# DAGroup-PKU/MHLA

Measured on AMD Instinct MI355X. Metric: MHLA fwd+bwd tokens/sec at (B,N,H,D), higher is better.
Workload: dtype bf16; 1 GPU; block-mix MHLA op fwd+bwd, per GPU B=8 N=4096 H=16 D=64 M=64 S=64 bf16 (BASELINE.json configs[1]); global_batch=8, parallelism=dp1 (batch shards, dW all-reduce only)

## Files before the change

### mhla_amd/csrc/capi_bm_typed.hpp

```cpp
#pragma once
#include "capi_common.hpp"
#include "blockmix.hpp"
#include "split.hpp"
#include "split16.hpp"
#include "mixh2.hpp"

namespace mhla {
namespace capi {

static_assert(sp::mixr_te<4, true>() == mixr_slice(true) && sp::mixr_te<4, false>() == mixr_slice(false), "bm_plan's resident-mixing rule");
template <int DT> constexpr int sp_state_threads() {
#ifdef MHLA_SP_STATE_4WAVES
    return NTHREADS;
#else
    return DT == 8 ? 512 : NTHREADS;
#endif
}
#ifndef SP_MIXH2_IH
#define SP_MIXH2_IH 2
#endif
#ifndef SP_MIXH2_RT
#define SP_MIXH2_RT 1
#endif

// ... 112 lines not shown
            break;
        case K_SP_MIXH: case K_SP_MIXH2:
            if constexpr (P24OK) return sp_mixh<TRANS>(o, p.mix[TRANS], p.nw, TRANS && p.dw_fused, wz, name, parts);
            break;
        default: break;
    }
    return fail(MHLA_EINVAL, "%s is not built for this type / head dim", name);
}
template <int TRANS>
int launch_wz(const float* W, int ldw, const float* x, float* out, int BH, int M, int S, float eps, hipStream_t st) {
    return launch(k_wz<TRANS>, dim3((S + 63) / 64, (M + 63) / 64, BH), dim3(NTHREADS), 0, st, N_WZ[TRANS], W, ldw, x, out, M, S, eps);
}

template <typename ET, int DT, int TRANS, bool S16>
int bm_state(const BmPlan& p, const BmCall& c, const StateArgs& a) {
    constexpr bool F32 = std::is_same<ET, float>::value;
    constexpr int SNT = sp_state_threads<DT>();
    const dim3 g(c.M, c.B * c.H);
    const char* name = p.n_state[TRANS];
    if (p.state == K_BM_STATE) return launch(k_bm_state<ET, DT, TRANS>, g, dim3(NTHREADS), state_smem_floats<DT>() * 4, c.st, name, a);
    if (p.state == K_S16_STATE) return launch(s16::k_s16_state<TRANS>, dim3((c.M + s16::WPB - 1) / s16::WPB, c.B * c.H), dim3(64 * s16::WPB), s16::state_smem(), c.st, name, a);
    if (p.rope) {
        if (p.fmt == SF_P24 || p.fmt == SF_H16) {
            if constexpr (F32 && bm_p24_built<ET, DT, S16>()) return launch(sp::k_sp_state<ET, DT, TRANS, true, SNT, false, 1>, g, dim3(SNT), sp::sp_state_smem<DT>(), c.st, name, a);
        } else if constexpr (F32 || TRANS == 0)
            return launch(sp::k_sp_state<ET, DT, TRANS, true, SNT, S16>, g, dim3(SNT), sp::sp_state_smem<DT>(), c.st, name, a);
        return MHLA_OK;
    }
    if constexpr (TRANS == 0 && bm_h16_built<ET, DT, S16>()) {
        if (p.fmt == SF_H16 && !(c.normalize && c.split) && g_recut.load())
            return launch(sp::k_sp_state<ET, DT, 0, false, SNT, S16, 2, false, false>, g, dim3(SNT), sp::sp_state_smem<DT>(), c.st, name, a);
    }
    WITH_PF(p.fmt, return launch(sp::k_sp_state<ET, DT, TRANS, false, SNT, S16, PF>, g, dim3(SNT),
                                 (PF && TRANS && sizeof(ET) == 2 && DT <= 4) ? sp::sp_state_rd_smem<DT>() : sp::sp_state_smem<DT>(), c.st, name, a));
    return MHLA_OK;
}
template <typename ET, int DT, bool S16>
int bm_state_and_mix(const BmPlan& p, const BmCall& c) {
    const BmWs& w = c.w;
    StateArgs a{};
    a.rcos = c.rcos; a.rsin = c.rsin; a.ldr = c.ldr;
    a.x = cv(c.k_num); a.y = cv(c.v); a.kd = cv(c.k_den); a.qd = cv(c.q_den); a.idx = c.block_index;
    a.out = w.kv; a.ksum = w.ksum; a.zo = w.z; a.es = w.es;
    a.H = c.H; a.M = c.M; a.S = c.S; a.D = c.D; a.eps = c.eps; a.relu = c.relu(); a.normalize = c.normalize; a.split = c.split;
    RC((bm_state<ET, DT, 0, S16>(p, c, a)));
    RC((bm_mix<0, S16, bm_p24_built<ET, DT, S16>()>(p, c)));
    if (p.wz_kernel) RC(launch_wz<0>(c.W, c.ldw, w.z, w.ninv, c.B * c.H, c.M, c.S, c.eps, c.st));
    return MHLA_OK;
}

template <typename ET, int DT, bool S16, typename TO = ET, bool EPI = false>
int sp_out(const BmPlan& p, const BmCall& c, const OutArgs& o, const char* name) {
    if constexpr (!EPI && bm_h16_built<ET, DT, S16>() && DT <= 4) {
        if (p.fmt == SF_H16 && bm_one_tile(c.S))
            return launch(sp::k_sp_out<ET, DT, TO, false, S16, 2, false, false, true>, dim3(c.M, c.B * c.H), dim3(sp::SP_OUT_T), sp::sp_out_smem<DT, S16>(), c.st, name, o);
    }
    WITH_PF(p.fmt, return launch(sp::k_sp_out<ET, DT, TO, EPI, S16, PF>, dim3(c.M, c.B * c.H), dim3(sp::SP_OUT_T), sp::sp_out_smem<DT, S16>(), c.st, name, o));
    return MHLA_OK;
}
inline OutArgs out_args(const BmCall& c) {
    OutArgs o{};
    o.rcos = c.rcos; o.rsin = c.rsin; o.ldr = c.ldr;
    o.q = cv(c.q_num); o.idx = c.block_index; o.W = c.W; o.ldw = c.ldw; o.g = c.w.g; o.ninv = c.w.ninv;
    o.H = c.H; o.M = c.M; o.S = c.S; o.D = c.D; o.eps = c.eps; o.es = c.w.es; o.relu = c.relu(); o.normalize = c.normalize;
    return o;
}
template <typename ET, int DT, bool S16>
// ... 48 lines not shown
    *parts = BH * nsplit;
    const DwArgs d{w.dg, w.kv, E, nullptr, nullptr, 0, w.dwp, M, tiles, nsplit, w.es};
    const dim3 g(p.dw_v ? 1 : tiles * tiles, BH, nsplit);
    if (p.dw == K_SP_DWT) {
        if constexpr (P24OK) return launch(sp::k_sp_dwt<true>, g, dim3(NTHREADS), sp::SP_DWT_SMEM, c.st, p.n_dw, d);
        return fail(MHLA_EINVAL, "%s is not built for this type / head dim", p.n_dw);
    }
    if (p.dw_v == 16) return launch(sp::k_sp_dw<S16, 1>, g, dim3(NTHREADS), sp::SP_DW_SMEM, c.st, p.n_dw, d);
    if (p.dw_v == 32) return launch(sp::k_sp_dw<S16, 2>, g, dim3(NTHREADS), sp::SP_DW_SMEM, c.st, p.n_dw, d);
    return launch(sp::k_sp_dw<S16>, g, dim3(NTHREADS), sp::SP_DW_SMEM, c.st, p.n_dw, d);
}
template <int MASK = 0>
int launch_dnz(const BmCall& c, int tiles, int parts) {
    const DwArgs dzz{c.w.dn, c.w.z, (long)c.S, nullptr, nullptr, 0, c.w.dwp + (size_t)parts * c.M * c.M, c.M, tiles, 1};
    return launch(k_dw<MASK>, dim3(tiles * tiles, c.B * c.H, 1), dim3(NTHREADS), DW_SMEM_FLOATS * 4, c.st, N_DNZ, dzz);
}
template <int MASK = 0>
int launch_dw_reduce(const float* dwp, float* dW, int M, int parts, int BH, bool el16, hipStream_t st) {
    if (el16 || M * M <= 1024 || parts >= 128) return launch(k_dw_reduce<MASK, 16>, dim3((M * M + 15) / 16), dim3(256), 0, st, N_DW_REDUCE, dwp, (const float*)nullptr, dW, M, M, parts, BH);
    return launch(k_dw_reduce<MASK>, dim3((M * M + 63) / 64), dim3(256), 0, st, N_DW_REDUCE, dwp, (const float*)nullptr, dW, M, M, parts, BH);
}

template <typename ET, int DT, bool S16>
int bm_tok(const BmPlan& p, const BmCall& c, const TokArgs& t) {
    const dim3 g(c.M, c.B * c.H), blk(NTHREADS);
    if (p.tok == K_BM_TOK) return launch(k_bm_bwd_tok<ET, DT>, g, blk, tok_smem_floats<DT>() * 4, c.st, p.n_tok[0], t);
    if (p.tok == K_S16_TOK) {
        const dim3 g16((c.M + s16::WPB - 1) / s16::WPB, c.B * c.H), b16(64 * s16::WPB);
        RC(launch(s16::k_s16_bwd_dq<0>, g16, b16, 0, c.st, p.n_tok[0], t));
        return launch(s16::k_s16_bwd_dkv<0>, g16, b16, s16::dkv_smem(), c.st, p.n_tok[1], t);
    }
    if (p.rope) {
        if constexpr (std::is_same<ET, float>::value) {
            WITH_PF(p.fmt, RC(launch(sp::k_sp_bwd_dq<ET, DT, true, false, false, PF>, g, blk, sp::sp_tok_smem<DT, false>(), c.st, p.n_tok[0], t));
                           return launch(sp::k_sp_bwd_dkv<ET, DT, true, false, PF>, g, blk, sp::sp_tok_smem<DT, false>(), c.st, p.n_tok[1], t));
        }
        return MHLA_OK;
    }
    const bool wq = c.normalize && !c.relu() && sizeof(ET) == 2 && DT != 5;
    constexpr bool ONE_BUILT = bm_h16_built<ET, DT, S16>() && DT <= 4;
    if (wq && ONE_BUILT && p.fmt == SF_H16 && bm_one_tile(c.S)) {
        if constexpr (ONE_BUILT) RC(launch(sp::k_sp_bwd_dq<ET, DT, false, S16, true, 2, true>, g, blk, sp::sp_tok_smem<DT, S16>(), c.st, p.n_tok[0], t));
    } else if (wq) WITH_PF(p.fmt, RC(launch(sp::k_sp_bwd_dq<ET, DT, false, S16, true, PF>, g, blk, sp::sp_tok_smem<DT, S16>(), c.st, p.n_tok[0], t)));
    else WITH_PF(p.fmt, RC(launch(sp::k_sp_bwd_dq<ET, DT, false, S16, false, PF>, g, blk, sp::sp_tok_smem<DT, S16>(), c.st, p.n_tok[0], t)));
    WITH_PF(p.fmt, return launch(sp::k_sp_bwd_dkv<ET, DT, false, S16, PF>, g, blk, sp::sp_tok_smem<DT, S16>(), c.st, p.n_tok[1], t));
    return MHLA_OK;
}

template <typename ET, bool S16>
int bm_fwd_typed(const BmCall& c) {
    const BmPlan p = bm_plan(c, false);
    DISPATCH_DT(dt_for(c.D), {
        RC((bm_state_and_mix<ET, DT, S16>(p, c)));
        OutArgs o = out_args(c);
        o.o = cmv(c.out);
        o.olo = (c.normalize && !c.epi && !(c.flags & MHLA_FLAG_NO_BWD_STATE)) ? c.w.olo : nullptr;
        RC((bm_out<ET, DT, S16>(p, c, o, p.n_out)));
    });
    return MHLA_OK;
}

template <typename ET, bool S16>
int bm_bwd_typed(const BmCall& c) {
    const BmPlan p = bm_plan(c, true);
    const BmWs& w = c.w;
    const int BH = c.B * c.H, M = c.M, S = c.S, tiles = (M + 63) / 64;
    DISPATCH_DT(dt_for(c.D), {
        if (!c.reuse) RC((bm_state_and_mix<ET, DT, S16>(p, c)));
        const bool want_olo = c.normalize && w.olo != nullptr, own_olo = !c.reuse || (c.flags & MHLA_FLAG_NO_BWD_STATE);
        if (want_olo && own_olo) {
            OutArgs o = out_args(c);
            o.o = MView{nullptr, 0, 0, 0}; o.olo = c.olo_own; o.skip_out = 1;
            RC((bm_out<ET, DT, S16>(p, c, o, p.n_olo)));
        }
        StateArgs a{};
        a.x = cv(c.q_num); a.y = cv(c.dout); a.o = cv(c.outv); a.idx = c.block_index; a.W = c.W; a.ldw = c.ldw; a.ninv = w.ninv;
        a.out = w.dg; a.dn = w.dn; a.es = w.es; a.H = c.H; a.M = M; a.S = S; a.D = c.D; a.eps = c.eps;
// ... 30 lines not shown
```

### mhla_amd/csrc/common.hpp

```cpp
#pragma once
#include <hip/hip_runtime.h>
#include <stdint.h>

namespace mhla {

typedef float f32x4 __attribute__((ext_vector_type(4)));
typedef float f32x2 __attribute__((ext_vector_type(2)));

struct bf16_t { unsigned short v; };
struct f16_t { _Float16 v; };

__device__ __forceinline__ float bf16_to_f32(unsigned short h) { return __uint_as_float(((unsigned)h) << 16); }
__device__ __forceinline__ unsigned short f32_to_bf16(float f) {
    unsigned u = __float_as_uint(f);
    if ((u & 0x7fffffffu) > 0x7f800000u) return (unsigned short)((u >> 16) | 0x40);
    u += 0x7fffu + ((u >> 16) & 1u);
    return (unsigned short)(u >> 16);
}

typedef __bf16 bf16x2_t __attribute__((ext_vector_type(2)));
__device__ __forceinline__ unsigned pack_bf16x2(float lo, float hi) {
    f32x2 v = {lo, hi};
    return __builtin_bit_cast(unsigned, __builtin_convertvector(v, bf16x2_t));
}
// ... 105 lines not shown

__device__ __forceinline__ float h16_mult_from_max(float mx) {
    const unsigned e = (__float_as_uint(mx) >> 23) & 0xffu;
    return __uint_as_float((e < 15u ? 1u : (e > 254u ? 240u : e - 14u)) << 23);
}
__device__ __forceinline__ float h16_mult_from_bound(float beta) {
    unsigned f = (__float_as_uint(beta) + 0x7fffffu) >> 23;
    f = f < 1u ? 1u : (f > 253u ? 253u : f);
    return __uint_as_float(f << 23);
}
__device__ __forceinline__ float h16_inv(float m) { return __uint_as_float(0x7f000000u - __float_as_uint(m)); }
typedef _Float16 h16x2_t __attribute__((ext_vector_type(2)));
__device__ __forceinline__ unsigned h16_pack2(float a, float b) {
    const h16x2_t h = {(_Float16)a, (_Float16)b};
    return __builtin_bit_cast(unsigned, h);
}
__device__ __forceinline__ uint4 h16_pack8(const f32x4& a, const f32x4& b, float inv) {
    return make_uint4(h16_pack2(a[0] * inv, a[1] * inv), h16_pack2(a[2] * inv, a[3] * inv), h16_pack2(b[0] * inv, b[1] * inv), h16_pack2(b[2] * inv, b[3] * inv));
}
__device__ __forceinline__ void h16_split8(const uint4& pay, float m, uint4& hi, uint4& lo) {
    const unsigned w[4] = {pay.x, pay.y, pay.z, pay.w};
    unsigned h[4], l[4];
#pragma unroll
    for (int j = 0; j < 4; ++j) {
        const h16x2_t p = __builtin_bit_cast(h16x2_t, w[j]);
        const float x0 = (float)p[0] * m, x1 = (float)p[1] * m;
        const unsigned u0 = __float_as_uint(x0), u1 = __float_as_uint(x1);
        h[j] = __builtin_amdgcn_perm(u1, u0, 0x07060302u);
        const float d0 = x0 - __uint_as_float(u0 & 0xffff0000u), d1 = x1 - __uint_as_float(u1 & 0xffff0000u);
        l[j] = __builtin_amdgcn_perm(__float_as_uint(d1), __float_as_uint(d0), 0x07060302u);
    }
    hi = make_uint4(h[0], h[1], h[2], h[3]);
    lo = make_uint4(l[0], l[1], l[2], l[3]);
}

struct View {
    const void* ptr;
    long sb, sn, sh;
};
struct MView {
    void* ptr;
    long sb, sn, sh;
};

__host__ __device__ constexpr int ld_kmajor(int dp) { return ((dp + 15) / 32) * 32 + 16; }
__host__ __device__ constexpr int ld_xmajor(int dp) { return dp + 2; }

__device__ __forceinline__ f32x4 mfma4(float a, float b, f32x4 c) {
    return __builtin_amdgcn_mfma_f32_16x16x4f32(a, b, c, 0, 0, 0);
}

__device__ __forceinline__ float wave_sum(float v) {
#pragma unroll
    for (int o = 32; o > 0; o >>= 1) v += __shfl_xor(v, o, 64);
    return v;
}

__device__ __forceinline__ float row16_sum(float v) {
    v += __int_as_float(__builtin_amdgcn_update_dpp(0, __float_as_int(v), 0x128, 0xf, 0xf, false));
    v += __int_as_float(__builtin_amdgcn_update_dpp(0, __float_as_int(v), 0x124, 0xf, 0xf, false));
    v += __int_as_float(__builtin_amdgcn_update_dpp(0, __float_as_int(v), 0x122, 0xf, 0xf, false));
    v += __int_as_float(__builtin_amdgcn_update_dpp(0, __float_as_int(v), 0x121, 0xf, 0xf, false));
    return v;
}

__device__ __forceinline__ long tok_row(const int* __restrict__ idx, long p) { return idx ? (long)idx[p] : p; }
// ... 90 lines not shown
```

### mhla_amd/csrc/split.hpp

```cpp
#pragma once
#include <type_traits>

#include "blockmix.hpp"
#include "fused.hpp"

namespace mhla {
namespace sp {

using fast::bf16x8;
using fast::mfma_bf16;
using fast::tr_read8;
using fast::s16x4;
using fast::s16x8;
using fast::u16;

__device__ __forceinline__ bf16x8 row_read8(const u16* tile, int ld, int c0, int k0, int lane);

template <typename T>
__device__ __forceinline__ void ld8(const T* p, f32x4& a, f32x4& b) {
    a = Io<T>::ld4(p);
    b = Io<T>::ld4(p + 4);
}
template <typename TO> struct Raw4 { typedef uint2 type; };
template <> struct Raw4<float> { typedef f32x4 type; };
// ... 151 lines not shown
                x[u][1] = gld<f32x4>(src + 4);
            }
        }
#pragma unroll
        for (int u = 0; u < UB; ++u) {
            const int r = r0 + RPP * (pb + u), off = mat_row<mat_new<DT>()>(r) * LD + cg;
            if (!(r < D && cg < D)) {
                x[u][0] = x[u][1] = f32x4{0.f, 0.f, 0.f, 0.f};
                x16[u] = make_uint4(0, 0, 0, 0);
                xl[u] = make_uint2(0, 0);
            }
            if (r < KP && cg < KP) {
                if (P24 == 2) {
                    uint4 hi, lo;
                    h16_split8(x16[u], hm, hi, lo);
                    *reinterpret_cast<uint4*>(Gh + off) = hi;
                    *reinterpret_cast<uint4*>(Gl + off) = lo;
                } else if (P24) {
                    *reinterpret_cast<uint4*>(Gh + off) = x16[u];
                    *reinterpret_cast<uint4*>(Gl + off) = p24_lo8(x16[u], xl[u]);
                } else if (S16) {
                    *reinterpret_cast<uint4*>(Gh + off) = x16[u];
                } else {
                    uint4 hi, lo;
                    split8(x[u][0], x[u][1], hi, lo);
                    *reinterpret_cast<uint4*>(Gh + off) = hi;
                    *reinterpret_cast<uint4*>(Gl + off) = lo;
                }
            }
        }
    }
}

template <int DT, int NT>
struct MatStage {
    static constexpr int PASSES = (Geo<DT>::KST * 32 + NT / Geo<DT>::CGS - 1) / (NT / Geo<DT>::CGS);
    uint4 x16[PASSES];
    uint2 xl[PASSES];
};
template <int DT, int NT>
__device__ __forceinline__ void stage_mat_issue(MatStage<DT, NT>& g, const float* __restrict__ base, long elem_off, int D, int tid, bool real = true) {
    constexpr int CGS = Geo<DT>::CGS, RPP = NT / CGS;
    const int r0 = tid / CGS, cg = (tid % CGS) * 8;
    const char* rowp = reinterpret_cast<const char*>(base + elem_off);
#pragma unroll
    for (int u = 0; u < MatStage<DT, NT>::PASSES; ++u) {
        const int r = min(r0 + RPP * u, D - 1), c = min(cg, D - 8), e = real ? r * D + c : 0;
        g.x16[u] = gld<uint4>(rowp + 2 * e);
        g.xl[u] = gld<uint2>(rowp + 2 * D * D + e);
    }
}
template <int DT, int NT>
__device__ __forceinline__ void stage_mat_commit(u16* __restrict__ Gh, u16* __restrict__ Gl, const MatStage<DT, NT>& g, int D, int tid) {
    constexpr int LD = mat_ld<DT>(), CGS = Geo<DT>::CGS, RPP = NT / CGS, KP = Geo<DT>::KST * 32;
    const int r0 = tid / CGS, cg = (tid % CGS) * 8;
#pragma unroll
    for (int u = 0; u < MatStage<DT, NT>::PASSES; ++u) {
        const int r = r0 + RPP * u, off = mat_row<mat_new<DT>()>(r) * LD + cg;
        const bool in = r < D && cg < D;
        const uint4 hi = in ? g.x16[u] : make_uint4(0, 0, 0, 0);
        const uint2 lo = in ? g.xl[u] : make_uint2(0, 0);
        if (r < KP && cg < KP) {
            *reinterpret_cast<uint4*>(Gh + off) = hi;
            *reinterpret_cast<uint4*>(Gl + off) = p24_lo8(hi, lo);
        }
    }
}

template <int DT>
__host__ __device__ constexpr int sp_state_smem() {
    static_assert(Geo<DT>::RPP * Geo<DT>::DW * 4 <= 4 * 32 * Geo<DT>::LD * 2, "column-sum partials must fit in the tiles");
    return 4 * 32 * Geo<DT>::LD * 2 + Geo<DT>::DW * 4;
}

template <int DT> __host__ __device__ constexpr int sp_state_rd_smem() {
    return 4 * 32 * Geo<DT>::LDR * 2 + Geo<DT>::DW * 4 + 2 * Geo<DT>::KST * 32 * mat_ld<DT>() * 2 + 2 * 32 * 4;
}

template <typename T, int DT, int MODE, bool ROPE = false, int NT = NTHREADS, bool S16 = Sum16<T>::value, int P24 = 0, bool PRO = false, bool TS = true>
__global__ __launch_bounds__(NT, NT == 512 ? 4 : (ROPE ? 2 : 3)) void k_sp_state(const StateArgs a) {
    static_assert(TS || MODE == 0, "the backward's third tensor is a property of its arithmetic (RD), not of the call");
    static_assert(!PRO || (MODE == 0 && !S16), "the prologue on load serves the forward's summary kernel");
    static_assert(!P24 || !S16, "p24 is a format of the fp32-grade summaries");
    constexpr bool RD = MODE == 1 && P24 && sizeof(T) == 2 && DT <= 4 && !ROPE;
    constexpr bool THIRD = TS && !RD;
    constexpr bool TN = !RD;
    constexpr int DW = Geo<DT>::DW, LD = TN ? Geo<DT>::LD : Geo<DT>::LDR, CGS = Geo<DT>::CGS, RPP = NT / CGS, IT = 32 / RPP, NWV = NT / 64,
                  RT = (DT + NWV - 1) / NWV, TILE = 32 * LD;
    static_assert(IT >= 1 && RPP * IT == 32, "a 32-row chunk must be whole staging passes");
    static_assert(RPP * DW * 4 <= 4 * 32 * LD * 2, "column-sum partials must fit in the tiles");
    constexpr bool LO = !std::is_same<T, bf16_t>::value || PRO;
    constexpr bool LOY = !std::is_same<T, bf16_t>::value || (MODE == 1 && !S16);
    constexpr int GLD = mat_ld<DT>(), GT = Geo<DT>::KST * 32 * GLD;
    extern __shared__ __attribute__((aligned(16))) unsigned char smem_raw[];
    u16* Kh = reinterpret_cast<u16*>(smem_raw);
    u16* Kl = Kh + TILE;
    u16* Vh = Kl + TILE;
    u16* Vl = Vh + TILE;
    float* cs = reinterpret_cast<float*>(smem_raw);
    float* vecd = reinterpret_cast<float*>(Vl + TILE);
    u16* Gh = reinterpret_cast<u16*>(vecd + DW);
    u16* Gl = Gh + GT;
    float* rdp = reinterpret_cast<float*>(Gl + GT);
    const int tid = threadIdx.x, wave = __builtin_amdgcn_readfirstlane(tid >> 6), lane = tid & 63, nl = lane & 15, kg = lane >> 4;
    const int blk = blockIdx.x, bh = blockIdx.y, b = bh / a.H, h = bh - b * a.H, S = a.S, D = a.D;
    const long p0 = (long)blk * S;
    const T* kb = (const T*)a.x.ptr + b * a.x.sb + h * a.x.sh;
    const T* vb = (const T*)a.y.ptr + b * a.y.sb + h * a.y.sh;
    const View& third = MODE == 0 ? a.kd : a.o;
    const T* kdb = (const T*)third.ptr + b * third.sb + h * third.sh;
    const bool den = THIRD && a.normalize && ((MODE == 1 && !RD) || (MODE == 0 && a.split));
    const int r0 = tid / CGS, cg = (tid % CGS) * 8;
    const float* ninvb = a.ninv + ((long)bh * a.M + blk) * S;

    typename Raw4<T>::type kr[IT][2], vr[IT][2], dr[THIRD ? IT : 1][2];
    f32x4 kx[IT][2], vx[IT][2], dx[THIRD ? IT : 1][2], rc[ROPE ? IT : 1], rs[ROPE ? IT : 1];
    float nv[IT];
    float prr[PRO ? IT : 1];
    f32x4 pw[PRO ? 2 : 1];
    constexpr bool rope = ROPE;
    int crow = 0;
    int nraw[IT], npos[IT];
    auto lookup = [&](int c0) __attribute__((always_inline)) {
#pragma unroll
        for (int it = 0; it < IT; ++it) {
            const long p = p0 + min(c0 + r0 + RPP * it, S - 1);
            nraw[it] = gld<int>(a.idx ? (const void*)(a.idx + p) : a.x.ptr);
            npos[it] = (int)p;
        }
    };
    lookup(0);
    const int cgc = min(cg, D - 8);
    if constexpr (PRO) {
        pw[0] = pw[1] = f32x4{1.f, 1.f, 1.f, 1.f};
        if (a.pro_wk) {
            pw[0] = *reinterpret_cast<const f32x4*>(a.pro_wk + h * D + cgc);
// ... 42 lines not shown
                vx[it][hf] = raw4_to_f32(T{}, vr[it][hf]);
                if constexpr (THIRD) dx[it][hf] = raw4_to_f32(T{}, dr[it][hf]);
            }
            if constexpr (PRO) {
                const float r = a.pro_rk ? prr[it] : 1.f;
                kx[it][0] = (kx[it][0] * r) * pw[0];
                kx[it][1] = (kx[it][1] * r) * pw[1];
            }
            if (a.relu) relu8(kx[it][0], kx[it][1], a.eps);
            kx[it][0] = valid ? kx[it][0] : z4; kx[it][1] = valid ? kx[it][1] : z4;
            vx[it][0] = valid ? vx[it][0] : z4; vx[it][1] = valid ? vx[it][1] : z4;
            if constexpr (THIRD) { dx[it][0] = (valid && den) ? dx[it][0] : z4; dx[it][1] = (valid && den) ? dx[it][1] : z4; }
            if constexpr (OLO) {
                const unsigned w[4] = {ox[it].x, ox[it].y, ox[it].z, ox[it].w};
                const bool on = valid && olo_on;
#pragma unroll
                for (int i = 0; i < 2; ++i) {
                    dx[it][0][2 * i] += on ? __uint_as_float(w[i] << 16) : 0.f;
                    dx[it][0][2 * i + 1] += on ? __uint_as_float(w[i] & 0xffff0000u) : 0.f;
                    dx[it][1][2 * i] += on ? __uint_as_float(w[2 + i] << 16) : 0.f;
                    dx[it][1][2 * i + 1] += on ? __uint_as_float(w[2 + i] & 0xffff0000u) : 0.f;
                }
            }
            nv[it] = (valid && MODE == 1 && a.normalize) ? nv[it] : 1.f;
            if constexpr (rope) {
                rc[it] = valid ? rc[it] : z4;
                rs[it] = valid ? rs[it] : z4;
            }
        }
    };
    float ksp[8] = {0.f, 0.f, 0.f, 0.f, 0.f, 0.f, 0.f, 0.f};
    float nvc[IT];
    int crowc = 0;
    auto commit = [&]() __attribute__((always_inline)) {
        __builtin_amdgcn_sched_barrier(0);
        settle();
#pragma unroll
        for (int it = 0; it < IT; ++it) {
            const int off = mat_row<TN>(r0 + RPP * it) * LD + cg;
            uint4 hi, lo;
            if (MODE == 1 && a.normalize) {
                if constexpr (THIRD) {
                    float d = 0.f;
#pragma unroll
                    for (int i = 0; i < 4; ++i) d += vx[it][0][i] * dx[it][0][i] + vx[it][1][i] * dx[it][1][i];
#pragma unroll
                    for (int o = CGS / 2; o > 0; o >>= 1) d += __shfl_xor(d, o, 64);
                    const int r = crow + r0 + RPP * it;
                    if (r < S && (tid % CGS) == 0) a.dn[((long)bh * a.M + blk) * S + r] = -d * nv[it];
                } else {
                    nvc[it] = nv[it];
                    crowc = crow;
                }
                vx[it][0] *= nv[it];
                vx[it][1] *= nv[it];
            }
            if constexpr (rope) {
                f32x4 r0 = kx[it][0], r1 = kx[it][1];
                rope8(r0, r1, rc[it], rs[it]);
                split8(r0, r1, hi, lo);
            } else {
                split8(kx[it][0], kx[it][1], hi, lo);
            }
            *reinterpret_cast<uint4*>(Kh + off) = hi;
            if (LO) *reinterpret_cast<uint4*>(Kl + off) = lo;
            split8(vx[it][0], vx[it][1], hi, lo);
            *reinterpret_cast<uint4*>(Vh + off) = hi;
            if (LOY) *reinterpret_cast<uint4*>(Vl + off) = lo;
            if (MODE == 0) {
                const f32x4* s = kx[it];
                if constexpr (THIRD) s = den ? dx[it] : kx[it];
#pragma unroll
                for (int i = 0; i < 4; ++i) {
                    ksp[i] += s[0][i];
                    ksp[4 + i] += s[1][i];
                }
            }
        }
    };

    f32x4 acc[RT][DT];
#pragma unroll
    for (int i = 0; i < RT; ++i)
#pragma unroll
        for (int j = 0; j < DT; ++j) acc[i][j] = f32x4{0.f, 0.f, 0.f, 0.f};

    fetch(0);
    if constexpr (RD) {
        if (a.normalize) stage_mat_split<DT, false, NT, P24>(Gh, Gl, a.g, ((long)bh * a.M + blk) * a.es, D, tid);
    }
    auto chunk = [&]<bool PF>(std::bool_constant<PF>, int c0) __attribute__((always_inline)) {
        commit();
        __syncthreads();
        if constexpr (PF) fetch(c0 + 32);
        if constexpr (RD) {
            if (a.normalize) {
                constexpr int KSTG = Geo<DT>::KST, CTH = (DT + 1) / 2;
                const int tt = wave & 1, hf = wave >> 1;
                bf16x8 bh_[KSTG], bl_[KSTG];
#pragma unroll
                for (int ks = 0; ks < KSTG; ++ks) {
                    bh_[ks] = mat_row_read8<TN>(Vh, LD, tt * 16, ks * 32, lane);
                    bl_[ks] = mat_row_read8<TN>(Vl, LD, tt * 16, ks * 32, lane);
                }
                float dot = 0.f;
#pragma unroll
                for (int c = 0; c < CTH; ++c) {
                    const int ct = hf * CTH + c;
                    if (ct < DT) {
                        f32x4 t4 = {0.f, 0.f, 0.f, 0.f};
#pragma unroll
                        for (int ks = 0; ks < KSTG; ++ks) {
                            const bf16x8 gh = mat_row_read8<mat_new<DT>()>(Gh, GLD, ct * 16, ks * 32, lane), gl = mat_row_read8<mat_new<DT>()>(Gl, GLD, ct * 16, ks * 32, lane);
                            t4 = mfma_bf16(gh, bh_[ks], t4);
                            t4 = mfma_bf16(gl, bh_[ks], t4);
                            t4 = mfma_bf16(gh, bl_[ks], t4);
                        }
                        const uint2 qr = *reinterpret_cast<const uint2*>(Kh + (tt * 16 + mat_row<TN>(nl)) * LD + ct * 16 + kg * 4);
                        f32x4 q4 = {__uint_as_float(qr.x << 16), __uint_as_float(qr.x & 0xffff0000u), __uint_as_float(qr.y << 16), __uint_as_float(qr.y & 0xffff0000u)};
                        if (LO) {
                            const uint2 ql = *reinterpret_cast<const uint2*>(Kl + (tt * 16 + mat_row<TN>(nl)) * LD + ct * 16 + kg * 4);
                            q4 += f32x4{__uint_as_float(ql.x << 16), __uint_as_float(ql.x & 0xffff0000u), __uint_as_float(ql.y << 16), __uint_as_float(ql.y & 0xffff0000u)};
                        }
                        dot += t4[0] * q4[0] + t4[1] * q4[1] + t4[2] * q4[2] + t4[3] * q4[3];
                    }
                }
                dot += __shfl_xor(dot, 16, 64);
                dot += __shfl_xor(dot, 32, 64);
                if (kg == 0) rdp[hf * 32 + tt * 16 + nl] = dot;
            }
        }
        bf16x8 ah[RT], al[RT];
#pragma unroll
        for (int rt = 0; rt < RT; ++rt) {
            const int c0 = min(wave * RT + rt, DW / 16 - 1) * 16;
            ah[rt] = mat_tr_read8<TN>(Kh, LD, 0, c0, lane);
            if (LO) al[rt] = mat_tr_read8<TN>(Kl, LD, 0, c0, lane);
        }
#pragma unroll
        for (int ct = 0; ct < DT; ++ct) {
            const bf16x8 bh_ = mat_tr_read8<TN>(Vh, LD, 0, ct * 16, lane);
#pragma unroll
            for (int rt = 0; rt < RT; ++rt) acc[rt][ct] = mfma_bf16(ah[rt], bh_, acc[rt][ct]);
            if (LOY) {
                const bf16x8 bl_ = mat_tr_read8<TN>(Vl, LD, 0, ct * 16, lane);
#pragma unroll
                for (int rt = 0; rt < RT; ++rt) acc[rt][ct] = mfma_bf16(ah[rt], bl_, acc[rt][ct]);
            }
            if (LO) {
// ... 1533 lines not shown
#pragma unroll
        for (int ks = 0; ks < CE / 32; ++ks) {
            bf16x8 ah[2], al[2], bh_[2], bl_[2];
#pragma unroll
            for (int t = 0; t < 2; ++t) {
                ah[t] = row_read8(Xh, LD, (2 * wi + t) * 16, ks * 32, lane);
                al[t] = row_read8(Xl, LD, (2 * wi + t) * 16, ks * 32, lane);
                bh_[t] = row_read8(Yh, LD, (2 * wj + t) * 16, ks * 32, lane);
                bl_[t] = row_read8(Yl, LD, (2 * wj + t) * 16, ks * 32, lane);
            }
#pragma unroll
            for (int i = 0; i < 2; ++i)
#pragma unroll
                for (int j = 0; j < 2; ++j) {
                    acc[i][j] = mfma_bf16(ah[i], bh_[j], acc[i][j]);
                    acc[i][j] = mfma_bf16(ah[i], bl_[j], acc[i][j]);
                    acc[i][j] = mfma_bf16(al[i], bh_[j], acc[i][j]);
                }
        }
        __syncthreads();
    }
    float* out = a.out + ((long)bh * a.nsplit + split) * M * M;
#pragma unroll
    for (int ti = 0; ti < 2; ++ti)
#pragma unroll
        for (int tj = 0; tj < 2; ++tj)
#pragma unroll
            for (int r = 0; r < 4; ++r) {
                const int i = i0 + 32 * wi + 16 * ti + 4 * kg + r, j = j0 + 32 * wj + 16 * tj + nl;
                if (i < M && j < M) out[(long)i * M + j] = acc[ti][tj][r];
            }
}

template <int DT, bool S16 = false>
__host__ __device__ constexpr int sp_tok_smem() {
    return sp_out_smem<DT, S16>() + Geo<DT>::DW * 4 * 4 + Geo<DT>::DW * 4 + (DT <= 4 ? 4 * 2 * 16 * (Geo<DT>::DW + 8) * 2 : 0);
}

__device__ __forceinline__ bf16x8 row_read8(const u16* tile, int ld, int c0, int k0, int lane) {
    return *reinterpret_cast<const bf16x8*>(tile + (c0 + (lane & 15)) * ld + k0 + (lane >> 4) * 8);
}

template <typename T, int DT, bool ROPE = false, bool S16 = Sum16<T>::value, bool WQ = false, int P24 = 0, bool ONE = false>
__global__ __launch_bounds__(NTHREADS, (DT <= 4 && WQ) ? 4 : 2) void k_sp_bwd_dq(const TokArgs a) {
    constexpr int LD = mat_ld<DT>(), DW = Geo<DT>::DW, KST = Geo<DT>::KST, TILE = KST * 32 * LD;
    extern __shared__ __attribute__((aligned(16))) unsigned char smem_raw[];
    u16* Gh = reinterpret_cast<u16*>(smem_raw);
    u16* Gl = Gh + TILE;
    float* dksw = reinterpret_cast<float*>(Gh + (S16 ? 1 : 2) * TILE);
    float* ksum = dksw + 4 * DW;
    const int tid = threadIdx.x, wave = __builtin_amdgcn_readfirstlane(tid >> 6), lane = tid & 63, nl = lane & 15, kg = lane >> 4;
    const int blk = blockIdx.x, bh = blockIdx.y, b = bh / a.H, h = bh - b * a.H, S = a.S, D = a.D, M = a.M;
    const long p0 = (long)blk * S;
    auto base = [&](const View& w) { return (const T*)w.ptr + b * w.sb + h * w.sh; };
    auto mbase = [&](const MView& w) { return (T*)w.ptr + b * w.sb + h * w.sh; };
    const T *gb = base(a.dout), *qdb = base(a.qd);
    T *dqb = mbase(a.dq), *dqdb = a.split ? mbase(a.dqd) : nullptr;
    const float* ninvb = a.ninv + ((long)bh * M + blk) * S;
    const float* dzb = a.dz + ((long)bh * M + blk) * S;
    constexpr bool wide_q = WQ;
    const bool wide_dq = view16(a.dq), wide_dqd = a.split && view16(a.dqd);

    struct Rows {
        typename Raw4<T>::type g[KST][2];
        typename Raw4<T>::type qd[WQ ? 1 : DT];
        typename Raw4<T>::type qw[WQ ? KST : 1][2];
        float ninv, dz;
        long row;
        bool live;
    } cur, nxt;
    const float* standin = a.g;
    auto look = [&](int tt) { return gld<int>(a.idx ? a.idx + p0 + min(tt * 16 + nl, S - 1) : reinterpret_cast<const int*>(a.g)); };
    auto fetch = [&](int tt, Rows& R, int looked) __attribute__((always_inline)) {
        const int s = tt * 16 + nl, sv = min(s, S - 1);
        R.live = s < S;
        R.row = a.idx ? (long)looked : p0 + sv;
        R.ninv = gld<float>(a.normalize ? ninvb + sv : standin);
        R.dz = gld<float>(a.normalize ? dzb + sv : standin);
        const T* grow = gb + R.row * a.dout.sn;
        const T* qrow = qdb + R.row * a.qd.sn;
#pragma unroll
        for (int ks = 0; ks < KST; ++ks) {
            const int c = ks * 32 + kg * 8 < D ? ks * 32 + kg * 8 : 0;
            R.g[ks][0] = gld<typename Raw4<T>::type>(grow + c);
            R.g[ks][1] = gld<typename Raw4<T>::type>(grow + c + 4);
        }
        if constexpr (!WQ) {
#pragma unroll
            for (int ct = 0; ct < DT; ++ct) R.qd[ct] = gld<typename Raw4<T>::type>(qrow + (ct * 16 + kg * 4 < D ? ct * 16 + kg * 4 : 0));
        }
        if constexpr (WQ) {
#pragma unroll
            for (int ks = 0; ks < KST; ++ks) {
                const int c = ks * 32 + kg * 8 < D ? ks * 32 + kg * 8 : 0;
                R.qw[ks][0] = gld<typename Raw4<T>::type>(qrow + c);
                R.qw[ks][1] = gld<typename Raw4<T>::type>(qrow + c + 4);
            }
        }
    };
    int lk = 0;
    if (a.idx) lk = gld<int>(a.idx + p0 + min(wave * 16 + nl, S - 1));
    fetch(wave, cur, lk);
    if constexpr (!ONE) lk = look(wave + 4);
    const float ksum_v = gld<float>(a.normalize ? a.ksum + ((long)bh * M + blk) * D + min(tid, D - 1) : standin);
    stage_mat_split<DT, S16, NTHREADS, P24>(Gh, Gl, a.g, ((long)bh * M + blk) * a.es, D, tid);
    if (tid < DW) ksum[tid] = (a.normalize && tid < D) ? ksum_v : 0.f;
    __syncthreads();
    f32x4 dksp[WQ ? 1 : DT], dksw8[WQ ? KST : 1][2];
#pragma unroll
    for (int ct = 0; ct < (WQ ? 1 : DT); ++ct) dksp[ct] = f32x4{0.f, 0.f, 0.f, 0.f};
#pragma unroll
    for (int ks = 0; ks < (WQ ? KST : 1); ++ks) dksw8[ks][0] = dksw8[ks][1] = f32x4{0.f, 0.f, 0.f, 0.f};

    auto tile = [&]() __attribute__((always_inline)) {
        const float cninv = a.normalize ? cur.ninv : 1.f, cdz = (a.normalize && cur.live) ? cur.dz : 0.f;
        bf16x8 gh[KST], gl[KST];
#pragma unroll
        for (int ks = 0; ks < KST; ++ks) {
            uint4 hi, lo;
            const bool in = ks * 32 + kg * 8 < D;
            const f32x4 z4 = {0.f, 0.f, 0.f, 0.f};
            split8((in ? raw4_to_f32(T{}, cur.g[ks][0]) : z4) * cninv, (in ? raw4_to_f32(T{}, cur.g[ks][1]) : z4) * cninv, hi, lo);
            gh[ks] = as_bf16x8(hi);
            gl[ks] = as_bf16x8(lo);
        }
        auto epilogue = [&](int ct, f32x4& c, f32x4& cd, const f32x2& rc, const f32x2& rs) {
            const int d0 = ct * 16 + kg * 4;
            if constexpr (ROPE) unrope4(c, rc, rs);
            f32x4 qd = {0.f, 0.f, 0.f, 0.f};
            if constexpr (!WQ) {
                if ((a.normalize || a.relu) && d0 < D) qd = raw4_to_f32(T{}, cur.qd[ct]);
            }
            if (a.relu)
#pragma unroll
                for (int i = 0; i < 4; ++i) qd[i] = fmaxf(qd[i], 0.f) + a.eps;
            const f32x4 ks4 = *reinterpret_cast<const f32x4*>(ksum + d0);
            cd = cdz * ks4;
            if (a.normalize) {
                if constexpr (!WQ) dksp[ct] += cdz * qd;
                if (!a.split) c += cd;
            }
            if (a.relu)
#pragma unroll
                for (int i = 0; i < 4; ++i)
                    if (!(qd[i] > a.eps)) c[i] = 0.f;
        };
#pragma unroll
        for (int ct = 0; ct < DT; ct += 2) {
            constexpr int LAST = DT - 1;
            const int c1t = ct + 1 <= LAST ? ct + 1 : LAST;
            f32x4 c0 = {0.f, 0.f, 0.f, 0.f}, c1 = c0;
            f32x2 rc0 = {1.f, 1.f}, rs0 = {0.f, 0.f}, rc1 = rc0, rs1 = rs0;
            if constexpr (ROPE) {
                const long ro = cur.row * a.ldr + kg * 2;
                if (ct * 16 + kg * 4 < D) { rc0 = *reinterpret_cast<const f32x2*>(a.rcos + ro + ct * 8); rs0 = *reinterpret_cast<const f32x2*>(a.rsin + ro + ct * 8); }
                if (c1t * 16 + kg * 4 < D) { rc1 = *reinterpret_cast<const f32x2*>(a.rcos + ro + c1t * 8); rs1 = *reinterpret_cast<const f32x2*>(a.rsin + ro + c1t * 8); }
            }
#pragma unroll
            for (int ks = 0; ks < KST; ++ks) {
                const bf16x8 a0h = mat_row_read8<mat_new<DT>()>(Gh, LD, ct * 16, ks * 32, lane), a1h = mat_row_read8<mat_new<DT>()>(Gh, LD, c1t * 16, ks * 32, lane);
                c0 = mfma_bf16(a0h, gh[ks], c0);
                c1 = mfma_bf16(a1h, gh[ks], c1);
                if (!S16) {
                    const bf16x8 a0l = mat_row_read8<mat_new<DT>()>(Gl, LD, ct * 16, ks * 32, lane), a1l = mat_row_read8<mat_new<DT>()>(Gl, LD, c1t * 16, ks * 32, lane);
                    c0 = mfma_bf16(a0l, gh[ks], c0);
                    c1 = mfma_bf16(a1l, gh[ks], c1);
                }
                c0 = mfma_bf16(a0h, gl[ks], c0);
                c1 = mfma_bf16(a1h, gl[ks], c1);
            }
            f32x4 e0, e1 = {0.f, 0.f, 0.f, 0.f};
            epilogue(ct, c0, e0, rc0, rs0);
            if (ct + 1 < DT) epilogue(ct + 1, c1, e1, rc1, rs1);
            store_tile_pair<T>(dqb + cur.row * a.dq.sn, ct, DT, D, kg, c0, c1, cur.live, wide_dq);
            if (a.normalize && a.split) store_tile_pair<T>(dqdb + cur.row * a.dqd.sn, ct, DT, D, kg, e0, e1, cur.live, wide_dqd);
            __builtin_amdgcn_sched_barrier(0);
        }
        if constexpr (WQ) {
#pragma unroll
            for (int ks = 0; ks < KST; ++ks) {
                const bool in = ks * 32 + kg * 8 < D;
                const f32x4 z4 = {0.f, 0.f, 0.f, 0.f};
                dksw8[ks][0] += cdz * (in ? raw4_to_f32(T{}, cur.qw[ks][0]) : z4);
                dksw8[ks][1] += cdz * (in ? raw4_to_f32(T{}, cur.qw[ks][1]) : z4);
            }
        }
    };
    if constexpr (ONE) {
        if (wave * 16 < S) tile();
    } else {
        for (int tt = wave; tt * 16 < S; tt += 4) {
            fetch((tt + 4) * 16 < S ? tt + 4 : tt, nxt, lk);
            lk = look(tt + 8);
            tile();
            cur = nxt;
        }
    }
    if (a.normalize) {
        if constexpr (WQ) {
#pragma unroll
            for (int ks = 0; ks < KST; ++ks)
#pragma unroll
// ... 225 lines not shown
```

Baseline: 96.85 million tokens/s.

## Use scaled fp16 payload operands instead of split bf16 hi/lo MFMAs in dq and state

```diff
diff --git a/mhla_amd/csrc/capi_bm_typed.hpp b/mhla_amd/csrc/capi_bm_typed.hpp
--- a/mhla_amd/csrc/capi_bm_typed.hpp
+++ b/mhla_amd/csrc/capi_bm_typed.hpp
@@ -168,7 +168,7 @@
             return launch(sp::k_sp_state<ET, DT, 0, false, SNT, S16, 2, false, false>, g, dim3(SNT), sp::sp_state_smem<DT>(), c.st, name, a);
     }
     WITH_PF(p.fmt, return launch(sp::k_sp_state<ET, DT, TRANS, false, SNT, S16, PF>, g, dim3(SNT),
-                                 (PF && TRANS && sizeof(ET) == 2 && DT <= 4) ? sp::sp_state_rd_smem<DT>() : sp::sp_state_smem<DT>(), c.st, name, a));
+                                 (PF && TRANS && sizeof(ET) == 2 && DT <= 4) ? sp::sp_state_rd_smem<DT, sp::sp_payrd<ET, DT, PF>()>() : sp::sp_state_smem<DT>(), c.st, name, a));
     return MHLA_OK;
 }
 template <typename ET, int DT, bool S16>
@@ -283,7 +283,7 @@
     }
     if (p.rope) {
         if constexpr (std::is_same<ET, float>::value) {
-            WITH_PF(p.fmt, RC(launch(sp::k_sp_bwd_dq<ET, DT, true, false, false, PF>, g, blk, sp::sp_tok_smem<DT, false>(), c.st, p.n_tok[0], t));
+            WITH_PF(p.fmt, RC(launch(sp::k_sp_bwd_dq<ET, DT, true, false, false, PF>, g, blk, sp::sp_dq_smem<DT, false, sp::sp_payop<ET, DT, PF, true>()>(), c.st, p.n_tok[0], t));
                            return launch(sp::k_sp_bwd_dkv<ET, DT, true, false, PF>, g, blk, sp::sp_tok_smem<DT, false>(), c.st, p.n_tok[1], t));
         }
         return MHLA_OK;
@@ -291,9 +291,9 @@
     const bool wq = c.normalize && !c.relu() && sizeof(ET) == 2 && DT != 5;
     constexpr bool ONE_BUILT = bm_h16_built<ET, DT, S16>() && DT <= 4;
     if (wq && ONE_BUILT && p.fmt == SF_H16 && bm_one_tile(c.S)) {
-        if constexpr (ONE_BUILT) RC(launch(sp::k_sp_bwd_dq<ET, DT, false, S16, true, 2, true>, g, blk, sp::sp_tok_smem<DT, S16>(), c.st, p.n_tok[0], t));
-    } else if (wq) WITH_PF(p.fmt, RC(launch(sp::k_sp_bwd_dq<ET, DT, false, S16, true, PF>, g, blk, sp::sp_tok_smem<DT, S16>(), c.st, p.n_tok[0], t)));
-    else WITH_PF(p.fmt, RC(launch(sp::k_sp_bwd_dq<ET, DT, false, S16, false, PF>, g, blk, sp::sp_tok_smem<DT, S16>(), c.st, p.n_tok[0], t)));
+        if constexpr (ONE_BUILT) RC(launch(sp::k_sp_bwd_dq<ET, DT, false, S16, true, 2, true>, g, blk, sp::sp_dq_smem<DT, S16, sp::sp_payop<ET, DT, 2>()>(), c.st, p.n_tok[0], t));
+    } else if (wq) WITH_PF(p.fmt, RC(launch(sp::k_sp_bwd_dq<ET, DT, false, S16, true, PF>, g, blk, sp::sp_dq_smem<DT, S16, sp::sp_payop<ET, DT, PF>()>(), c.st, p.n_tok[0], t)));
+    else WITH_PF(p.fmt, RC(launch(sp::k_sp_bwd_dq<ET, DT, false, S16, false, PF>, g, blk, sp::sp_dq_smem<DT, S16, sp::sp_payop<ET, DT, PF>()>(), c.st, p.n_tok[0], t)));
     WITH_PF(p.fmt, return launch(sp::k_sp_bwd_dkv<ET, DT, false, S16, PF>, g, blk, sp::sp_tok_smem<DT, S16>(), c.st, p.n_tok[1], t));
     return MHLA_OK;
 }
diff --git a/mhla_amd/csrc/common.hpp b/mhla_amd/csrc/common.hpp
--- a/mhla_amd/csrc/common.hpp
+++ b/mhla_amd/csrc/common.hpp
@@ -161,6 +161,30 @@
     }
     hi = make_uint4(h[0], h[1], h[2], h[3]);
     lo = make_uint4(l[0], l[1], l[2], l[3]);
+}
+
+typedef _Float16 f16x8 __attribute__((ext_vector_type(8)));
+template <int FIRST = 16, int LANES = 4>
+__device__ __forceinline__ float tok16_scale(float lane_max) {
+    float mx = lane_max;
+#pragma unroll
+    for (int o = FIRST; o < FIRST * LANES; o <<= 1) mx = fmaxf(mx, __shfl_xor(mx, o, 64));
+    const unsigned e = (__float_as_uint(mx) >> 23) & 0xffu;
+    unsigned f = 268u - e;
+    f = f > 253u ? 253u : f;
+    return __uint_as_float((mx == 0.f ? 127u : f) << 23);
+}
+template <int NP>
+__device__ __forceinline__ float tok16_operands(const f32x4 (&x)[NP][2], f16x8 (&op)[NP]) {
+    float mx = 0.f;
+#pragma unroll
+    for (int p = 0; p < NP; ++p)
+#pragma unroll
+        for (int i = 0; i < 4; ++i) mx = fmaxf(mx, fmaxf(fabsf(x[p][0][i]), fabsf(x[p][1][i])));
+    const float u = tok16_scale(mx);
+#pragma unroll
+    for (int p = 0; p < NP; ++p) op[p] = __builtin_bit_cast(f16x8, h16_pack8(x[p][0], x[p][1], u));
+    return u;
 }
 
 struct View {
diff --git a/mhla_amd/csrc/split.hpp b/mhla_amd/csrc/split.hpp
--- a/mhla_amd/csrc/split.hpp
+++ b/mhla_amd/csrc/split.hpp
@@ -207,6 +207,32 @@
     }
 }
 
+#ifndef SP_PAYLOAD_OPERANDS
+#define SP_PAYLOAD_OPERANDS 1
+#endif
+template <typename T, int DT, int P24, bool ROPE = false>
+__host__ __device__ constexpr bool sp_payop() { return SP_PAYLOAD_OPERANDS && P24 == 2 && sizeof(T) == 2 && DT <= 4 && !ROPE; }
+template <int DT, int NT = NTHREADS>
+__device__ __forceinline__ float stage_mat_payload(u16* __restrict__ G, const float* __restrict__ base, long elem_off, int D, int tid) {
+    constexpr int LD = mat_ld<DT>(), CGS = Geo<DT>::CGS, RPP = NT / CGS, KP = Geo<DT>::KST * 32;
+    const int r0 = tid / CGS, cg = (tid % CGS) * 8;
+    constexpr int PASSES = (KP + RPP - 1) / RPP;
+    const char* rowp = reinterpret_cast<const char*>(base + elem_off);
+    const float hm = gld<float>(rowp + 2 * D * D);
+    uint4 x16[PASSES];
+#pragma unroll
+    for (int u = 0; u < PASSES; ++u) {
+        const int r = min(r0 + RPP * u, D - 1), c = min(cg, D - 8);
+        x16[u] = gld<uint4>(rowp + 2 * (r * D + c));
+    }
+#pragma unroll
+    for (int u = 0; u < PASSES; ++u) {
+        const int r = r0 + RPP * u;
+        if (r < KP && cg < KP) *reinterpret_cast<uint4*>(G + mat_row<mat_new<DT>()>(r) * LD + cg) = (r < D && cg < D) ? x16[u] : make_uint4(0, 0, 0, 0);
+    }
+    return hm;
+}
+
 template <int DT, int NT>
 struct MatStage {
     static constexpr int PASSES = (Geo<DT>::KST * 32 + NT / Geo<DT>::CGS - 1) / (NT / Geo<DT>::CGS);
@@ -248,9 +274,12 @@
     return 4 * 32 * Geo<DT>::LD * 2 + Geo<DT>::DW * 4;
 }
 
-template <int DT> __host__ __device__ constexpr int sp_state_rd_smem() {
-    return 4 * 32 * Geo<DT>::LDR * 2 + Geo<DT>::DW * 4 + 2 * Geo<DT>::KST * 32 * mat_ld<DT>() * 2 + 2 * 32 * 4;
-}
+template <int DT, bool ONEP = false> __host__ __device__ constexpr int sp_state_rd_smem() {
+    return 4 * 32 * (ONEP ? Geo<DT>::LD : Geo<DT>::LDR) * 2 + Geo<DT>::DW * 4 + (ONEP ? 1 : 2) * Geo<DT>::KST * 32 * mat_ld<DT>() * 2 + 2 * 32 * 4;
+}
+template <typename T, int DT, int P24>
+__host__ __device__ constexpr bool sp_payrd() { return sp_payop<T, DT, P24>() && std::is_same<T, bf16_t>::value; }
+static_assert(!SP_PAYLOAD_OPERANDS || 5 * sp_state_rd_smem<4, true>() <= 160 * 1024, "five k_sp_state<1> (row dots from G) workgroups per CU at D = 64");
 
 template <typename T, int DT, int MODE, bool ROPE = false, int NT = NTHREADS, bool S16 = Sum16<T>::value, int P24 = 0, bool PRO = false, bool TS = true>
 __global__ __launch_bounds__(NT, NT == 512 ? 4 : (ROPE ? 2 : 3)) void k_sp_state(const StateArgs a) {
@@ -259,7 +288,8 @@
     static_assert(!P24 || !S16, "p24 is a format of the fp32-grade summaries");
     constexpr bool RD = MODE == 1 && P24 && sizeof(T) == 2 && DT <= 4 && !ROPE;
     constexpr bool THIRD = TS && !RD;
-    constexpr bool TN = !RD;
+    constexpr bool PAYRD = RD && sp_payrd<T, DT, P24>();
+    constexpr bool TN = !RD || PAYRD;
     constexpr int DW = Geo<DT>::DW, LD = TN ? Geo<DT>::LD : Geo<DT>::LDR, CGS = Geo<DT>::CGS, RPP = NT / CGS, IT = 32 / RPP, NWV = NT / 64,
                   RT = (DT + NWV - 1) / NWV, TILE = 32 * LD;
     static_assert(IT >= 1 && RPP * IT == 32, "a 32-row chunk must be whole staging passes");
@@ -276,7 +306,7 @@
     float* vecd = reinterpret_cast<float*>(Vl + TILE);
     u16* Gh = reinterpret_cast<u16*>(vecd + DW);
     u16* Gl = Gh + GT;
-    float* rdp = reinterpret_cast<float*>(Gl + GT);
+    float* rdp = reinterpret_cast<float*>(Gh + (PAYRD ? 1 : 2) * GT);
     const int tid = threadIdx.x, wave = __builtin_amdgcn_readfirstlane(tid >> 6), lane = tid & 63, nl = lane & 15, kg = lane >> 4;
     const int blk = blockIdx.x, bh = blockIdx.y, b = bh / a.H, h = bh - b * a.H, S = a.S, D = a.D;
     const long p0 = (long)blk * S;
@@ -385,6 +415,7 @@
     float ksp[8] = {0.f, 0.f, 0.f, 0.f, 0.f, 0.f, 0.f, 0.f};
     float nvc[IT];
     int crowc = 0;
+    float gm = 1.f;
     auto commit = [&]() __attribute__((always_inline)) {
         __builtin_amdgcn_sched_barrier(0);
         settle();
@@ -404,6 +435,14 @@
                 } else {
                     nvc[it] = nv[it];
                     crowc = crow;
+                    if constexpr (PAYRD) {
+                        float mx = 0.f;
+#pragma unroll
+                        for (int i = 0; i < 4; ++i) mx = fmaxf(mx, fmaxf(fabsf(vx[it][0][i]), fabsf(vx[it][1][i])));
+                        const float u = tok16_scale<1, CGS>(mx);
+                        *reinterpret_cast<uint4*>(Kl + off) = h16_pack8(vx[it][0], vx[it][1], u);
+                        nvc[it] = ((gm * nv[it]) * h16_inv(u)) * nv[it];
+                    }
                 }
                 vx[it][0] *= nv[it];
                 vx[it][1] *= nv[it];
@@ -440,7 +479,10 @@
 
     fetch(0);
     if constexpr (RD) {
-        if (a.normalize) stage_mat_split<DT, false, NT, P24>(Gh, Gl, a.g, ((long)bh * a.M + blk) * a.es, D, tid);
+        if (a.normalize) {
+            if constexpr (PAYRD) gm = stage_mat_payload<DT, NT>(Gh, a.g, ((long)bh * a.M + blk) * a.es, D, tid);
+            else stage_mat_split<DT, false, NT, P24>(Gh, Gl, a.g, ((long)bh * a.M + blk) * a.es, D, tid);
+        }
     }
     auto chunk = [&]<bool PF>(std::bool_constant<PF>, int c0) __attribute__((always_inline)) {
         commit();
@@ -453,8 +495,8 @@
                 bf16x8 bh_[KSTG], bl_[KSTG];
 #pragma unroll
                 for (int ks = 0; ks < KSTG; ++ks) {
-                    bh_[ks] = mat_row_read8<TN>(Vh, LD, tt * 16, ks * 32, lane);
-                    bl_[ks] = mat_row_read8<TN>(Vl, LD, tt * 16, ks * 32, lane);
+                    bh_[ks] = mat_row_read8<TN>(PAYRD ? Kl : Vh, LD, tt * 16, ks * 32, lane);
+                    if constexpr (!PAYRD) bl_[ks] = mat_row_read8<TN>(Vl, LD, tt * 16, ks * 32, lane);
                 }
                 float dot = 0.f;
 #pragma unroll
@@ -464,10 +506,15 @@
                         f32x4 t4 = {0.f, 0.f, 0.f, 0.f};
 #pragma unroll
                         for (int ks = 0; ks < KSTG; ++ks) {
-                            const bf16x8 gh = mat_row_read8<mat_new<DT>()>(Gh, GLD, ct * 16, ks * 32, lane), gl = mat_row_read8<mat_new<DT>()>(Gl, GLD, ct * 16, ks * 32, lane);
-                            t4 = mfma_bf16(gh, bh_[ks], t4);
-                            t4 = mfma_bf16(gl, bh_[ks], t4);
-                            t4 = mfma_bf16(gh, bl_[ks], t4);
+                            const bf16x8 gh = mat_row_read8<mat_new<DT>()>(Gh, GLD, ct * 16, ks * 32, lane);
+                            if constexpr (PAYRD) {
+                                t4 = fast::mfma_f16(fast::as_f16x8(gh), fast::as_f16x8(bh_[ks]), t4);
+                            } else {
+                                const bf16x8 gl = mat_row_read8<mat_new<DT>()>(Gl, GLD, ct * 16, ks * 32, lane);
+                                t4 = mfma_bf16(gh, bh_[ks], t4);
+                                t4 = mfma_bf16(gl, bh_[ks], t4);
+                                t4 = mfma_bf16(gh, bl_[ks], t4);
+                            }
                         }
                         const uint2 qr = *reinterpret_cast<const uint2*>(Kh + (tt * 16 + mat_row<TN>(nl)) * LD + ct * 16 + kg * 4);
                         f32x4 q4 = {__uint_as_float(qr.x << 16), __uint_as_float(qr.x & 0xffff0000u), __uint_as_float(qr.y << 16), __uint_as_float(qr.y & 0xffff0000u)};
@@ -2067,9 +2114,14 @@
             }
 }
 
+template <int DT, bool S16 = false, bool ONEP = false>
+__host__ __device__ constexpr int sp_dq_smem() {
+    return ((S16 || ONEP) ? 1 : 2) * Geo<DT>::KST * 32 * mat_ld<DT>() * 2 + Geo<DT>::DW * 4 * 4 + Geo<DT>::DW * 4;
+}
+static_assert(6 * sp_dq_smem<4, false, false>() <= 160 * 1024 && 6 * sp_dq_smem<4, false, true>() <= 160 * 1024, "six k_sp_bwd_dq workgroups per CU at D = 64");
 template <int DT, bool S16 = false>
 __host__ __device__ constexpr int sp_tok_smem() {
-    return sp_out_smem<DT, S16>() + Geo<DT>::DW * 4 * 4 + Geo<DT>::DW * 4 + (DT <= 4 ? 4 * 2 * 16 * (Geo<DT>::DW + 8) * 2 : 0);
+    return sp_dq_smem<DT, S16>() + (DT <= 4 ? 4 * 2 * 16 * (Geo<DT>::DW + 8) * 2 : 0);
 }
 
 __device__ __forceinline__ bf16x8 row_read8(const u16* tile, int ld, int c0, int k0, int lane) {
@@ -2080,9 +2132,10 @@
 __global__ __launch_bounds__(NTHREADS, (DT <= 4 && WQ) ? 4 : 2) void k_sp_bwd_dq(const TokArgs a) {
     constexpr int LD = mat_ld<DT>(), DW = Geo<DT>::DW, KST = Geo<DT>::KST, TILE = KST * 32 * LD;
     extern __shared__ __attribute__((aligned(16))) unsigned char smem_raw[];
+    constexpr bool PAYOP = sp_payop<T, DT, P24, ROPE>();
     u16* Gh = reinterpret_cast<u16*>(smem_raw);
     u16* Gl = Gh + TILE;
-    float* dksw = reinterpret_cast<float*>(Gh + (S16 ? 1 : 2) * TILE);
+    float* dksw = reinterpret_cast<float*>(Gh + ((S16 || PAYOP) ? 1 : 2) * TILE);
     float* ksum = dksw + 4 * DW;
     const int tid = threadIdx.x, wave = __builtin_amdgcn_readfirstlane(tid >> 6), lane = tid & 63, nl = lane & 15, kg = lane >> 4;
     const int blk = blockIdx.x, bh = blockIdx.y, b = bh / a.H, h = bh - b * a.H, S = a.S, D = a.D, M = a.M;
@@ -2138,7 +2191,9 @@
     fetch(wave, cur, lk);
     if constexpr (!ONE) lk = look(wave + 4);
     const float ksum_v = gld<float>(a.normalize ? a.ksum + ((long)bh * M + blk) * D + min(tid, D - 1) : standin);
-    stage_mat_split<DT, S16, NTHREADS, P24>(Gh, Gl, a.g, ((long)bh * M + blk) * a.es, D, tid);
+    float gm = 1.f;
+    if constexpr (PAYOP) gm = stage_mat_payload<DT>(Gh, a.g, ((long)bh * M + blk) * a.es, D, tid);
+    else stage_mat_split<DT, S16, NTHREADS, P24>(Gh, Gl, a.g, ((long)bh * M + blk) * a.es, D, tid);
     if (tid < DW) ksum[tid] = (a.normalize && tid < D) ? ksum_v : 0.f;
     __syncthreads();
     f32x4 dksp[WQ ? 1 : DT], dksw8[WQ ? KST : 1][2];
@@ -2150,14 +2205,28 @@
     auto tile = [&]() __attribute__((always_inline)) {
         const float cninv = a.normalize ? cur.ninv : 1.f, cdz = (a.normalize && cur.live) ? cur.dz : 0.f;
         bf16x8 gh[KST], gl[KST];
-#pragma unroll
-        for (int ks = 0; ks < KST; ++ks) {
-            uint4 hi, lo;
-            const bool in = ks * 32 + kg * 8 < D;
-            const f32x4 z4 = {0.f, 0.f, 0.f, 0.f};
-            split8((in ? raw4_to_f32(T{}, cur.g[ks][0]) : z4) * cninv, (in ? raw4_to_f32(T{}, cur.g[ks][1]) : z4) * cninv, hi, lo);
-            gh[ks] = as_bf16x8(hi);
-            gl[ks] = as_bf16x8(lo);
+        f16x8 g16[KST];
+        float cscale = 1.f;
+        if constexpr (PAYOP) {
+            f32x4 x[KST][2];
+#pragma unroll
+            for (int ks = 0; ks < KST; ++ks) {
+                const bool in = ks * 32 + kg * 8 < D;
+                const f32x4 z4 = {0.f, 0.f, 0.f, 0.f};
+                x[ks][0] = in ? raw4_to_f32(T{}, cur.g[ks][0]) : z4;
+                x[ks][1] = in ? raw4_to_f32(T{}, cur.g[ks][1]) : z4;
+            }
+            cscale = (gm * cninv) * h16_inv(tok16_operands<KST>(x, g16));
+        } else {
+#pragma unroll
+            for (int ks = 0; ks < KST; ++ks) {
+                uint4 hi, lo;
+                const bool in = ks * 32 + kg * 8 < D;
+                const f32x4 z4 = {0.f, 0.f, 0.f, 0.f};
+                split8((in ? raw4_to_f32(T{}, cur.g[ks][0]) : z4) * cninv, (in ? raw4_to_f32(T{}, cur.g[ks][1]) : z4) * cninv, hi, lo);
+                gh[ks] = as_bf16x8(hi);
+                gl[ks] = as_bf16x8(lo);
+            }
         }
         auto epilogue = [&](int ct, f32x4& c, f32x4& cd, const f32x2& rc, const f32x2& rs) {
             const int d0 = ct * 16 + kg * 4;
@@ -2194,15 +2263,24 @@
 #pragma unroll
             for (int ks = 0; ks < KST; ++ks) {
                 const bf16x8 a0h = mat_row_read8<mat_new<DT>()>(Gh, LD, ct * 16, ks * 32, lane), a1h = mat_row_read8<mat_new<DT>()>(Gh, LD, c1t * 16, ks * 32, lane);
-                c0 = mfma_bf16(a0h, gh[ks], c0);
-                c1 = mfma_bf16(a1h, gh[ks], c1);
-                if (!S16) {
-                    const bf16x8 a0l = mat_row_read8<mat_new<DT>()>(Gl, LD, ct * 16, ks * 32, lane), a1l = mat_row_read8<mat_new<DT>()>(Gl, LD, c1t * 16, ks * 32, lane);
-                    c0 = mfma_bf16(a0l, gh[ks], c0);
-                    c1 = mfma_bf16(a1l, gh[ks], c1);
-                }
-                c0 = mfma_bf16(a0h, gl[ks], c0);
-                c1 = mfma_bf16(a1h, gl[ks], c1);
+                if constexpr (PAYOP) {
+                    c0 = fast::mfma_f16(fast::as_f16x8(a0h), g16[ks], c0);
+                    c1 = fast::mfma_f16(fast::as_f16x8(a1h), g16[ks], c1);
+                } else {
+                    c0 = mfma_bf16(a0h, gh[ks], c0);
+                    c1 = mfma_bf16(a1h, gh[ks], c1);
+                    if (!S16) {
+                        const bf16x8 a0l = mat_row_read8<mat_new<DT>()>(Gl, LD, ct * 16, ks * 32, lane), a1l = mat_row_read8<mat_new<DT>()>(Gl, LD, c1t * 16, ks * 32, lane);
+                        c0 = mfma_bf16(a0l, gh[ks], c0);
+                        c1 = mfma_bf16(a1l, gh[ks], c1);
+                    }
+                    c0 = mfma_bf16(a0h, gl[ks], c0);
+                    c1 = mfma_bf16(a1h, gl[ks], c1);
+                }
+            }
+            if constexpr (PAYOP) {
+                c0 *= cscale;
+                c1 *= cscale;
             }
             f32x4 e0, e1 = {0.f, 0.f, 0.f, 0.f};
             epilogue(ct, c0, e0, rc0, rs0);
```

Result: faster. 99.66 million tokens/s, median of 6 (+2.9%).
